# Gaurav14cs17/Bayer_Low_light_Image_Enhancement

Hardware: AMD Instinct MI355X
Metric: megapixels/sec RawFormer-S 512x512 RAW->sRGB (higher is better)
Workload: dtype f32; 1 GPU; RawFormer-S(FLCA) dim=32, batch=8 of packed 4x512x512 synthetic Bayer per GPU; frames_per_gpu=8, variant=flca, weights=synthetic (seeded, random-init scale), parallelism=batch-sharded x1, device=AMD Radeon Graphics

## Files before the change

### bayer_low_light_image_enhancement_amd/_lib.py

```python
from __future__ import annotations

import ctypes as C
import os

_HERE = os.path.dirname(os.path.abspath(__file__))
LIB_PATH = os.environ.get("RF_LIB_PATH") or os.path.join(_HERE, "csrc", "librawformer_hip.so")

RF_VARIANT_FLCA = 0
RF_VARIANT_PLAIN = 1
RF_VARIANT_TRUECOLOR = 2


class RfConfig(C.Structure):
    _fields_ = [("dim", C.c_int32), ("heads", C.c_int32 * 4), ("inp_channels", C.c_int32),
                ("out_channels", C.c_int32), ("ffn_expansion", C.c_int32), ("variant", C.c_int32),
                ("branch_lrelu", C.c_int32), ("clamp_io", C.c_int32), ("flca_levels", C.c_int32)]


_vp, _i, _f, _sz = C.c_void_p, C.c_int, C.c_float, C.c_size_t
ALLREDUCE_FN = C.CFUNCTYPE(None, C.c_void_p, C.c_void_p, C.c_size_t, C.c_int, C.c_void_p)
_psz = C.POINTER(C.c_size_t)
GRAD_READY_FN = C.CFUNCTYPE(None, C.c_void_p, C.c_size_t, C.c_size_t, C.c_void_p)

SIGNATURES = {
    "rf_last_error": (C.c_char_p, []),
    "rf_version": (_i, []),
    "rf_profile_begin": (_i, []),
    "rf_profile_end": (_i, [C.c_char_p, _sz]),
    "rf_create": (_i, [C.POINTER(RfConfig), C.POINTER(_vp)]),
    "rf_destroy": (None, [_vp]),
    "rf_param_count": (_i, [_vp]),
    "rf_param_info": (_i, [_vp, _i, C.POINTER(C.c_char_p), C.POINTER(C.c_int64 * 4), C.POINTER(_i)]),
    "rf_set_param": (_i, [_vp, C.c_char_p, _vp, C.POINTER(C.c_int64), _i]),
    "rf_packed_bytes": (_i, [_vp, _psz]),
    "rf_pack_params": (_i, [_vp, _vp, _sz, _vp]),
    "rf_workspace_bytes": (_i, [_vp, _i, _i, _i, _psz]),
    "rf_forward": (_i, [_vp, _vp, _vp, _vp, _sz, _i, _i, _i, _i, _vp]),
    "rf_forward_stage": (_i, [_vp, _i, _vp, _vp, _vp, _vp, _sz, _i, _i, _i, _vp]),
    "rf_set_shard": (_i, [_vp, _i, _i, _i, ALLREDUCE_FN, _vp]),
    "rf_set_shard_grid": (_i, [_vp, _i, _i, _i, _i, _i, _i, ALLREDUCE_FN, _vp]),
    "rf_flat_param_floats": (_i, [_vp, _psz]),
    "rf_flat_offset": (_i, [_vp, _i, _psz]),
    "rf_train_workspace_bytes": (_i, [_vp, _i, _i, _i, _psz]),
    "rf_set_grad_ready": (_i, [_vp, GRAD_READY_FN, _vp]),
    "rf_set_loss_clamp": (_i, [_vp, _i]),
    "rf_grad_range_count": (_i, [_vp, C.POINTER(_i)]),
    "rf_grad_range": (_i, [_vp, _i, _psz, _psz]),
    "rf_train_step": (_i, [_vp, _vp, _vp, _vp, _vp, _vp, _vp, _sz, _i, _i, _i, _i, _f, _vp]),
    "rf_adam_step": (_i, [_vp, _vp, _vp, _vp, _sz, _f, _f, _f, _f, _f, _i, _i, _f, _vp]),
    "rf_pixel_unshuffle2": (_i, [_vp, _vp, _i, _i, _i, _i, _vp]),
    "rf_pixel_shuffle2": (_i, [_vp, _vp, _i, _i, _i, _i, _vp]),
    "rf_dwt_haar": (_i, [_vp, _vp, _i, _i, _i, _i, _vp]),
    "rf_idwt_haar": (_i, [_vp, _vp, _i, _i, _i, _i, _vp]),
    "rf_dwt_custom": (_i, [_vp, _vp, C.POINTER(C.c_float), _i, _i, _i, _i, _i, _vp]),
    "rf_idwt_custom": (_i, [_vp, _vp, C.POINTER(C.c_float), _i, _i, _i, _i, _i, _vp]),
    "rf_haar_dwt": (_i, [_vp, _vp, _i, _i, _i, _i, _vp]),
    "rf_layernorm2d": (_i, [_vp, _vp, _vp, _vp, _f, _i, _i, _i, _i, _vp]),
    "rf_conv1x1_scratch_bytes": (_i, [_i, _i, _psz]),
    "rf_conv1x1": (_i, [_vp, _vp, _vp, _vp, _vp, _vp, _vp, _vp, _vp, _i, _i, _i, _i, _i, _i, _vp]),
    "rf_dwconv3x3": (_i, [_vp, _vp, _vp, _vp, _i, _i, _i, _i, _i, _vp]),
    "rf_conv3x3_scratch_bytes": (_i, [_i, _i, _psz]),
    "rf_conv3x3": (_i, [_vp, _vp, _vp, _vp, _vp, _i, _i, _i, _i, _i, _i, _i, _vp]),
    "rf_convT2x2_scratch_bytes": (_i, [_i, _i, _psz]),
    "rf_convT2x2": (_i, [_vp, _vp, _vp, _vp, _vp, _i, _i, _i, _i, _i, _vp]),
    "rf_chan_attn_scratch_bytes": (_i, [_i, _i, _i, _i, _i, _psz]),
    "rf_chan_attn": (_i, [_vp] * 10 + [_i] * 5 + [_vp]),
    "rf_transformer_block_scratch_bytes": (_i, [_i, _i, _i, _i, _i, _i, _psz]),
    "rf_transformer_block": (_i, [_vp, _vp, C.POINTER(_vp), _vp, _i, _i, _i, _i, _i, _i, _vp]),
    "rf_flca_scratch_bytes": (_i, [_i, _i, _i, _i, _psz]),
    "rf_flca": (_i, [_vp, _vp, _vp, C.POINTER(_vp), _vp, _i, _i, _i, _i, _vp]),
    "rf_guidance_scratch_bytes": (_i, [_i, _i, _i, _psz]),
    "rf_flca_guidance": (_i, [_vp, _vp, _vp, _i, _i, _i, _i, _i, _vp]),
    "rf_to_uint8_hwc": (_i, [_vp, _vp, _i, _i, _i, _i, _vp]),
    "rf_u8_sse": (_i, [_vp, _vp, _vp, _i, _sz, _vp]),
    "rf_u8_channel_sums": (_i, [_vp, _vp, _i, _i, _sz, _vp]),
    "rf_u8_ssim_scratch_bytes": (_i, [_i, _i, _i, _i, _psz]),
    "rf_u8_ssim": (_i, [_vp, _vp, _vp, _vp, _i, _i, _i, _i, _vp]),
    "rf_sid_pack": (_i, [_vp, _vp, _i, _i, _i, _i, _i, C.c_double, _i, _vp]),
    "rf_sid_check_desc": (_i, [C.POINTER(C.c_int), _i, _i, _i, _i, _i, _i]),
    "rf_sid_sample": (_i, [_vp, _vp, _vp, _vp, _vp, _vp, _i, _i, _i, _i, _i, _i, _i, _i, _vp]),
    "rf_mcr_sample": (_i, [_vp, _vp, _vp, _vp, _vp, _vp, _i, _i, _i, _i, _i, _i, _vp]),
    "rf_token_attn": (_i, [_vp, _vp, _vp, _vp, C.c_longlong, C.c_longlong, _i, _i, _i, _i, _f, _vp]),
    "rf_bayer_luma_scratch_bytes": (_i, [_i, _i, _i, _psz]),
    "rf_bayer_luma": (_i, [_vp, _vp, _vp, _i, _i, _i, _i, _vp]),
    "rf_luma_film_scratch_bytes": (_i, [_i, _i, _i, _psz]),
    "rf_luma_film": (_i, [_vp, _vp, _vp, C.c_longlong, _vp, _vp, _vp, _vp, _i, _i, _i, _i, _vp]),
    "rf_dwgate3x3": (_i, [_vp, _vp, _vp, _vp, _vp, _vp, _i, _i, _i, _i, _vp]),
    "rf_dwconv5x5": (_i, [_vp, _vp, _vp, _vp, _i, _i, _i, _i, _vp]),
    "rf_rfft2_polar_scratch_bytes": (_i, [_i, _i, _i, _psz]),
    "rf_rfft2_polar": (_i, [_vp, _vp, _vp, _vp, _i, _i, _i, _vp]),
    "rf_polar_irfft2": (_i, [_vp, _vp, _vp, _vp, _i, _i, _i, _vp]),
    "rf_feb_scratch_bytes": (_i, [_i, _i, _i, _i, _psz]),
    "rf_feb": (_i, [_vp, _vp, C.POINTER(_vp), _vp, _i, _i, _i, _i, _vp]),
    "rf_ffab_scratch_bytes": (_i, [_i, _i, _i, _i, _psz]),
    "rf_ffab": (_i, [_vp, _vp, C.POINTER(_vp), _vp, _i, _i, _i, _i, _vp]),
    "rf_affine_clamp_add": (_i, [_vp, _vp, _vp, _sz, _f, _f, _f, _f, _vp]),
    "rf_upcat_scratch_bytes": (_i, [_i, _psz]),
    "rf_upcat": (_i, [_vp] * 8 + [_i, _i, _i, _i, _vp]),
}

_lib = None


def load() -> C.CDLL:
    global _lib
    if _lib is None:
        if not os.path.exists(LIB_PATH):
            raise RuntimeError(
                f"{LIB_PATH} not found: build it with `python -m bayer_low_light_image_enhancement_amd.build` "
                "(hipcc, gfx950).  There is no CPU fallback for the RawFormer HIP path.")
        lib = C.CDLL(LIB_PATH)
        for name, (res, args) in SIGNATURES.items():
# ... 12 lines not shown
```

### bayer_low_light_image_enhancement_amd/csrc/rf_api.hip

```cpp
#include <cstdarg>
#include <cstdio>
#include <cstring>
#include <map>
#include <string>
#include <vector>
#include "rf_common.h"

namespace rf {

static thread_local char g_err[512] = "";

void set_error(const char* fmt, ...) {
    va_list ap;
    va_start(ap, fmt);
    vsnprintf(g_err, sizeof(g_err), fmt, ap);
    va_end(ap);
}

int check_hip(hipError_t e, const char* what) {
    if (e == hipSuccess) return RF_OK;
    set_error("%s: %s", what, hipGetErrorString(e));
    return RF_E_DEVICE;
}

// ... 81 lines not shown
    return launch_pixel_unshuffle2(in, out, B, C, h, w, (hipStream_t)stream);
}

int rf_pixel_shuffle2(const float* in, float* out, int B, int C, int h, int w, void* stream) {
    RF_CHECK_ARG(in && out && B > 0 && C > 0 && h > 0 && w > 0, "pixel_shuffle2: bad arguments");
    return launch_pixel_shuffle2(in, out, B, C, h, w, (hipStream_t)stream);
}

int rf_dwt_haar(const float* in, float* out, int B, int C, int h, int w, void* stream) {
    RF_CHECK_ARG(in && out && B > 0 && C > 0 && h > 0 && w > 0, "dwt_haar: bad arguments");
    return launch_dwt2x2(in, out, kHaarInit, 0, 1, B, C, h, w, 2 * h, 2 * w, (hipStream_t)stream);
}

int rf_idwt_haar(const float* in, float* out, int B, int C, int h, int w, void* stream) {
    RF_CHECK_ARG(in && out && B > 0 && C > 0 && h > 0 && w > 0, "idwt_haar: bad arguments");
    return launch_idwt2x2(in, out, kHaarInit, 0, 1, B, C, h, w, (hipStream_t)stream);
}

static void scaled_kernel(const float* k16, int norm, float out[16]) {
    for (int i = 0; i < 16; ++i) out[i] = norm ? k16[i] / 2.0f : k16[i];
}

int rf_dwt_custom(const float* in, float* out, const float* k16, int norm, int B, int C, int h, int w, void* stream) {
    RF_CHECK_ARG(in && out && k16 && B > 0 && C > 0 && h > 0 && w > 0, "dwt_custom: bad arguments");
    float k[16];
    scaled_kernel(k16, norm, k);
    return launch_dwt2x2(in, out, k, 1, 0, B, C, h, w, 2 * h, 2 * w, (hipStream_t)stream);
}

int rf_idwt_custom(const float* in, float* out, const float* k16, int norm, int B, int C, int h, int w, void* stream) {
    RF_CHECK_ARG(in && out && k16 && B > 0 && C > 0 && h > 0 && w > 0, "idwt_custom: bad arguments");
    float k[16];
    scaled_kernel(k16, norm, k);
    return launch_idwt2x2(in, out, k, 1, 0, B, C, h, w, (hipStream_t)stream);
}

int rf_haar_dwt(const float* in, float* out, int B, int C, int hin, int win, void* stream) {
    RF_CHECK_ARG(in && out && B > 0 && C > 0 && hin > 1 && win > 1, "haar_dwt: bad arguments");
    return launch_dwt2x2(in, out, kHaarOrtho, 0, 0, B, C, (hin + 1) / 2, (win + 1) / 2, hin, win, (hipStream_t)stream);
}

int rf_layernorm2d(const float* in, float* out, const float* weight, const float* bias, float eps,
                   int B, int C, int h, int w, void* stream) {
    RF_CHECK_ARG(in && out && weight && B > 0 && C > 0 && h > 0 && w > 0, "layernorm2d: bad arguments");
    return launch_layernorm2d(in, out, weight, bias, eps, B, C, h * w, (hipStream_t)stream);
}

int rf_conv1x1_scratch_bytes(int Cin_total, int Cout, size_t* bytes) {
    RF_CHECK_ARG(bytes && Cin_total > 0 && Cout > 0, "conv1x1_scratch_bytes: bad arguments");
    *bytes = (align_up(packed1x1_floats(Cin_total, Cout), 64) + packed1x1_b3_floats(Cin_total, Cout)) * sizeof(float);
    return RF_OK;
}

int rf_conv1x1(const float* in, const float* in2, float* out, const float* weight, const float* bias,
               const float* ln_w, const float* ln_b, const float* res, void* scratch,
               int B, int C1, int C2, int Cout, int h, int w, void* stream) {
    RF_CHECK_ARG(in && out && weight && scratch && aligned16(scratch), "conv1x1: bad arguments");
    hipStream_t st = (hipStream_t)stream;
    const int K = C1 + C2;
    RF_TRY(pack_1x1(weight, (float*)scratch, Cout, K, K, 1, st));
    float* w3 = (float*)scratch + align_up(packed1x1_floats(K, Cout), 64);
    RF_TRY(pack_1x1_b3(weight, w3, Cout, K, K, 1, st));
    Conv1x1Args a{};
    a.x1 = in; a.C1 = C1; a.x1_bstride = (int64_t)C1 * h * w;
    a.x2 = C2 ? in2 : nullptr; a.C2 = C2; a.x2_bstride = (int64_t)C2 * h * w;
    a.wp = (const float*)scratch; a.wp3 = w3; a.bias = bias; a.ln_w = ln_w; a.ln_b = ln_b; a.ln_eps = 1e-5f;
    a.res = res; a.res_bstride = (int64_t)Cout * h * w;
    a.out = out; a.out_bstride = (int64_t)Cout * h * w; a.Cout = Cout; a.B = B; a.P = h * w; a.w = w;
    return launch_conv1x1(a, st);
}

int rf_dwconv3x3(const float* in, float* out, const float* weight, const float* bias, int gelu,
                 int B, int C, int h, int w, void* stream) {
    RF_CHECK_ARG(in && out && weight && B > 0 && C > 0 && h > 0 && w > 0, "dwconv3x3: bad arguments");
    DwConvArgs a{};
    a.x = in; a.x_bstride = (int64_t)C * h * w; a.out = out; a.out_bstride = (int64_t)C * h * w;
    a.w = weight; a.bias = bias; a.B = B; a.C = C; a.h = h; a.w_ = w; a.gelu = gelu;
    return launch_dwconv3x3(a, (hipStream_t)stream);
}

int rf_conv3x3_scratch_bytes(int Cin, int Cout, size_t* bytes) {
    RF_CHECK_ARG(bytes && Cin > 0 && Cout > 0, "conv3x3_scratch_bytes: bad arguments");
    *bytes = packed3x3_floats(Cin, Cout) * sizeof(float);
    return RF_OK;
}

int rf_conv3x3(const float* in, float* out, const float* weight, const float* bias, void* scratch,
               int act, int store, int B, int Cin, int Cout, int h, int w, void* stream) {
    RF_CHECK_ARG(in && out && weight && scratch && aligned16(scratch), "conv3x3: bad arguments");
    hipStream_t st = (hipStream_t)stream;
    RF_TRY(pack_3x3(weight, (float*)scratch, Cout, Cin, st));
    Conv3x3Args a{};
    a.x = in; a.x_bstride = (int64_t)Cin * h * w; a.wp = (const float*)scratch; a.bias = bias;
    a.out = out; a.out_bstride = (int64_t)Cout * h * w; a.B = B; a.Cin = Cin; a.Cout = Cout; a.h = h; a.w = w;
    a.act = act; a.store = store;
    return launch_conv3x3(a, st);
}

int rf_convT2x2_scratch_bytes(int Cin, int Cout, size_t* bytes) {
    RF_CHECK_ARG(bytes && Cin > 0 && Cout > 0, "convT2x2_scratch_bytes: bad arguments");
    *bytes = packed1x1_floats(Cin, 4 * Cout) * sizeof(float);
    return RF_OK;
}

int rf_convT2x2(const float* in, float* out, const float* weight, const float* bias, void* scratch,
                int B, int Cin, int Cout, int h, int w, void* stream) {
// ... 169 lines not shown
```

### bayer_low_light_image_enhancement_amd/csrc/rf_common.h

```cpp
#pragma once
#include <hip/hip_runtime.h>
#include <stdint.h>
#include <stddef.h>
#include "../../include/rawformer_hip.h"

namespace rf {

typedef float f32x4 __attribute__((ext_vector_type(4)));

void set_error(const char* fmt, ...);
int check_hip(hipError_t e, const char* what);
int check_launch(const char* what);

#define RF_CHECK_ARG(cond, ...)            \
    do {                                   \
        if (!(cond)) {                     \
            rf::set_error(__VA_ARGS__);    \
            return RF_E_INVALID;           \
        }                                  \
    } while (0)

#define RF_TRY(expr)            \
    do {                        \
        const int rc_ = (expr); \
// ... 80 lines not shown
#undef RF_B3
}
#endif

int pack_1x1(const float* w, float* packed, int Cout, int K, int64_t row_stride, int64_t col_stride, hipStream_t st);
int pack_3x3(const float* w, float* packed, int Cout, int Cin, hipStream_t st);
int pack_convT(const float* w, float* packed, int Cin, int Cout, hipStream_t st);

struct PackDesc {
    const float* src; float* dst;
    int kind;
    int rows, cols;
    int64_t rs, cs;
    int flip;
};
constexpr int kPackBatch = 48;
struct PackBatch { PackDesc d[kPackBatch]; };
size_t pack_desc_floats(const PackDesc& d);
int launch_pack_batch(const PackDesc* d, int n, hipStream_t st);

size_t upcat_packed_floats(int C);
int pack_upcat(const float* up_w, const float* up_b, const float* cr_w, const float* cr_b, float* packed, int C, hipStream_t st);
bool upcat_supported(int C, int h, int w, const void* x, const void* skip, const void* out);
int launch_upcat(const float* x, const float* skip, float* out, const float* packed, int B, int C, int h, int w, hipStream_t st);

struct Conv1x1Args {
    const float* x1;
    const float* x2;
    int C1, C2;
    int64_t x1_bstride;
    int64_t x2_bstride;
    const float* x3;
    int C3;
    int64_t x3_bstride;
    const float* wp;
    int64_t wp_bstride;
    const void* wp3;
    int64_t wp3_bstride;
    const float* bias;
    const float* ln_w;
    const float* ln_b;
    float ln_eps;
    const float* res;
    int64_t res_bstride;
    float* out;
    int64_t out_bstride;
    int Cout;
    int B, P;
    int w;
    int mode;
    int act;
};
int launch_conv1x1(const Conv1x1Args& a, hipStream_t st);
bool conv1x1_ln_single_pass(const Conv1x1Args& a);

struct Conv3x3Args {
    const float* x;
    int64_t x_bstride;
    const float* wp;
    const float* bias;
    float* out;
    int64_t out_bstride;
    int B, Cin, Cout, h, w;
    int act;
    int store;
    int unshuffle_in;
    int clamp_in;
    int clamp_out;
    float* ks_scratch = nullptr;
    size_t ks_floats = 0;
};
int launch_conv3x3(const Conv3x3Args& a, hipStream_t st);
size_t conv3x3_ksplit_floats(int B, int Cout, int h, int w);
size_t conv3x3_ksplit_counter_bytes();

template <class T> struct SeGroup { T se1_w, se1_b, se3_w, se3_b; };
template <class T> struct FlcaGroup {
    T alpha, beta, gamma;
    T w_low, w_high, w_chr;
    SeGroup<T> se;
};
typedef SeGroup<const float*> SePrm;
typedef FlcaGroup<const float*> FlcaPrm;
typedef FlcaGroup<float*> FlcaGrad;
static inline int flca_hidden(int C) { return C / 8 > 8 ? C / 8 : 8; }

int launch_layernorm2d(const float* in, float* out, const float* w, const float* b, float eps,
                       int B, int C, int P, hipStream_t st);
struct DwConvArgs {
    const float* x; int64_t x_bstride;
    float* out; int64_t out_bstride;
    const float* w;
    const float* bias;
    int B, C, h, w_;
    int gelu;
    float* out2 = nullptr;
};
int launch_dwconv3x3(const DwConvArgs& a, hipStream_t st);
int launch_pixel_unshuffle2(const float* in, float* out, int B, int C, int h, int w, hipStream_t st);
int launch_pixel_shuffle2(const float* in, float* out, int B, int C, int h, int w, hipStream_t st);
int launch_dwt2x2(const float* in, float* out, const float k[16], int layout, int exact_haar,
                  int B, int C, int h, int w, int hin, int win, hipStream_t st);
int launch_idwt2x2(const float* in, float* out, const float k[16], int layout, int exact_haar,
                   int B, int C, int h, int w, hipStream_t st);

struct GramArgs {
// ... 196 lines not shown
```

### bayer_low_light_image_enhancement_amd/csrc/rf_gemm1x1.hip

```cpp
#include <cstdio>
#include <cstdlib>
#include "rf_common.h"

namespace rf {

__device__ __forceinline__ const float* kset_base(const Conv1x1Args& a, int b, int s) {
    const int k = 4 * s;
    const bool first = k < a.C1;
    const float* src = first ? a.x1 : a.x2;
    const size_t off = (size_t)b * (size_t)(first ? a.x1_bstride : a.x2_bstride) + (size_t)(first ? k : k - a.C1) * (size_t)a.P;
    return src + off;
}

__device__ __forceinline__ float4 ldv(const float* __restrict__ base, unsigned off) {
    return *reinterpret_cast<const float4*>(base + off);
}

template <int NCO, bool RES>
__device__ __forceinline__ void epilogue(const Conv1x1Args& a, f32x4 (&acc)[NCO][4], int tfirst, int ntiles,
                                         const float* __restrict__ bias_l, const float4* res,
                                         int b, int p0, int kq, bool live) {
    const int P = a.P;
    float* outb = a.out + (size_t)b * a.out_bstride;
    if (a.mode == 0) {
// ... 315 lines not shown
    auto chunk = [&](int c, float4 (&xc)[KCH], float4 (&xn)[KCH]) {
        if (c + 1 < nch) {
            load_x_chunk(c + 1, xn);
            load_w_chunk(c + 1);
        }
        const float* wl = &lds_w[c & 1][lane];
#pragma unroll
        for (int i = 0; i < KCH; ++i) {
            float xv[4] = {xc[i].x, xc[i].y, xc[i].z, xc[i].w};
            if constexpr (LN) {
                const int k = 4 * (c * KCH + i) + kq;
                const float gk = gam_l[k], bk = bet_l[k];
#pragma unroll
                for (int g = 0; g < 4; ++g) xv[g] = fmaf(fmaf(xv[g], lnA[g], lnB[g]), gk, bk);
            }
#pragma unroll
            for (int t = 0; t < NCO; ++t) {
                const float av = wl[(i * NCO + t) * 64];
#pragma unroll
                for (int g = 0; g < 4; ++g)
                    acc[t][g] = __builtin_amdgcn_mfma_f32_16x16x4f32(av, xv[g], acc[t][g], 0, 0, 0);
            }
        }
        if (c + 1 < nch) store_w_chunk((c + 1) & 1);
        __syncthreads();
    };

    load_x_chunk(0, xa);
    load_w_chunk(0);
    store_w_chunk(0);
    __syncthreads();
    for (int c = 0; c < nch; c += 2) {
        chunk(c, xa, xb_);
        if (c + 1 < nch) chunk(c + 1, xb_, xa);
    }
    epilogue<NCO, false>(a, acc, t0, tcnt, bias_l, nullptr, b, p0, kq, live);
}


__device__ __forceinline__ void b3_load_x_block(float4 (&xr)[8], const float* xb1, const float* xb2, const float* xb3, int C1, int C2, int C3,
                                                int c, int kq, unsigned P, unsigned pl) {
    const int cb = 32 * c;
    const bool first = cb < C1, third = cb >= C1 + C2;
    const float* src = first ? xb1 : third ? xb3 : xb2;
    const int cloc = first ? cb : third ? cb - C1 - C2 : cb - C1, cmax = (first ? C1 : third ? C3 : C2) - 1;
#pragma unroll
    for (int i = 0; i < 8; ++i) {
        int ch = cloc + 8 * kq + i;
        ch = ch < cmax ? ch : cmax;
        xr[i] = ldv(src, (unsigned)ch * P + pl);
    }
}

template <int NCO, bool LN>
__global__ void __launch_bounds__(256, 2) conv1x1_b3_kernel(Conv1x1Args a, int ngroups) {
    __shared__ __attribute__((aligned(16))) u32x4 lds_w[2][NCO * 3 * 64];
    __shared__ float bias_l[NCO * 16];
    __shared__ float gam_l[LN ? kStreamLnMaxK : 4], bet_l[LN ? kStreamLnMaxK : 4];
    constexpr int WPT = (NCO * 3 * 64 + 255) / 256;
    const int tid = threadIdx.x;
    const int lane = tid & 63, wave = tid >> 6;
    const int j = lane & 15, kq = lane >> 4;
    const int grp = blockIdx.x % ngroups;
    const int tile = blockIdx.x / ngroups;
    const int b = blockIdx.y;
    const int P = a.P;
    const int K = a.C1 + a.C2 + a.C3;
    const int NB = (K + 31) >> 5;
    const int NT = (a.Cout + 15) >> 4;
    const int t0 = grp * NCO;
    const int tcnt = (NT - t0 < NCO) ? NT - t0 : NCO;
    const int p0 = (tile * 4 + wave) * 64 + 4 * j;
    const bool live = p0 < P;
    const unsigned pl = (unsigned)(live ? p0 : 0);
    const u32x4* wp3 = reinterpret_cast<const u32x4*>(reinterpret_cast<const float*>(a.wp3) + (size_t)b * a.wp3_bstride);
    stage_bias(a, bias_l, t0, NCO, tid);
    if constexpr (LN) {
        for (int i = tid; i < 32 * NB; i += 256) {
            gam_l[i] = i < K ? a.ln_w[i] : 0.f;
            bet_l[i] = (a.ln_b && i < K) ? a.ln_b[i] : 0.f;
        }
    }

    f32x4 acc[NCO][4];
#pragma unroll
    for (int t = 0; t < NCO; ++t)
#pragma unroll
        for (int g = 0; g < 4; ++g) acc[t][g] = (f32x4){0.f, 0.f, 0.f, 0.f};
    if (a.res && a.mode == 0) {
        const float* resb = a.res + (size_t)b * a.res_bstride;
#pragma unroll
        for (int t = 0; t < NCO; ++t)
#pragma unroll
            for (int r = 0; r < 4; ++r) {
                const int co = 16 * (t0 + t) + 4 * kq + r;
                const bool ok = live && t < tcnt && co < a.Cout;
                const float4 rv = ldv(resb + (size_t)(ok ? co : 0) * P, pl);
                acc[t][0][r] = ok ? rv.x : 0.f; acc[t][1][r] = ok ? rv.y : 0.f;
                acc[t][2][r] = ok ? rv.z : 0.f; acc[t][3][r] = ok ? rv.w : 0.f;
            }
    }

    float lnA[4] = {1.f, 1.f, 1.f, 1.f}, lnB[4] = {0.f, 0.f, 0.f, 0.f};
    if constexpr (LN) {
        const unsigned voff = (unsigned)kq * (unsigned)P + pl;
        const float4 s4 = ldv(kset_base(a, b, 0), pl);
        const float sh[4] = {s4.x, s4.y, s4.z, s4.w};
        float s1[4] = {0.f, 0.f, 0.f, 0.f}, s2[4] = {0.f, 0.f, 0.f, 0.f};
#pragma unroll 16
        for (int s = 0; s < (K >> 2); ++s) {
            const float4 t = ldv(kset_base(a, b, s), voff);
            const float d[4] = {t.x - sh[0], t.y - sh[1], t.z - sh[2], t.w - sh[3]};
#pragma unroll
            for (int g = 0; g < 4; ++g) { s1[g] += d[g]; s2[g] = fmaf(d[g], d[g], s2[g]); }
        }
        const float invK = 1.0f / (float)K;
#pragma unroll
        for (int g = 0; g < 4; ++g) {
            s1[g] += __shfl_xor(s1[g], 16); s1[g] += __shfl_xor(s1[g], 32);
            s2[g] += __shfl_xor(s2[g], 16); s2[g] += __shfl_xor(s2[g], 32);
            const float md = s1[g] * invK;
            const float var = fmaxf(fmaf(-md, md, s2[g] * invK), 0.f);
            const float rstd = 1.0f / sqrtf(var + a.ln_eps);
            lnA[g] = rstd;
            lnB[g] = a.ln_b ? -(sh[g] + md) * rstd : 0.f;
        }
    }

    float4 xr[8];
    u32x4 wr[WPT];
    const float* const xb1 = a.x1 + (size_t)b * (size_t)a.x1_bstride;
    const float* const xb2 = a.x2 + (size_t)b * (size_t)a.x2_bstride;
    const float* const xb3 = a.x3 + (size_t)b * (size_t)a.x3_bstride;
    auto load_x_block = [&](int c) { b3_load_x_block(xr, xb1, xb2, xb3, a.C1, a.C2, a.C3, c, kq, (unsigned)P, pl); };
    auto load_w_block = [&](int c) {
#pragma unroll
        for (int i = 0; i < WPT; ++i) {
            const int idx = tid + 256 * i;
            const int t = idx / 192, rem = idx - t * 192;
            const bool ok = idx < NCO * 192 && t < tcnt;
            const u32x4 v = wp3[((size_t)c * NT + t0 + (ok ? t : 0)) * 192 + (ok ? rem : 0)];
            wr[i] = ok ? v : (u32x4){0u, 0u, 0u, 0u};
        }
    };
    auto store_w_block = [&](int buf) {
#pragma unroll
        for (int i = 0; i < WPT; ++i)
            if (tid + 256 * i < NCO * 192) lds_w[buf][tid + 256 * i] = wr[i];
    };

    load_x_block(0);
    load_w_block(0);
    store_w_block(0);
    __syncthreads();
    for (int c = 0; c < NB; ++c) {
        u32x4 bp[4][3];
#pragma unroll
        for (int hp = 0; hp < 4; ++hp) {
            float xa[4] = {xr[2 * hp].x, xr[2 * hp].y, xr[2 * hp].z, xr[2 * hp].w};
            float xb[4] = {xr[2 * hp + 1].x, xr[2 * hp + 1].y, xr[2 * hp + 1].z, xr[2 * hp + 1].w};
            if constexpr (LN) {
                const int k = 32 * c + 8 * kq + 2 * hp;
                const float ga = gam_l[k], ba = bet_l[k], gb = gam_l[k + 1], bb = bet_l[k + 1];
#pragma unroll
                for (int g = 0; g < 4; ++g) {
                    xa[g] = fmaf(fmaf(xa[g], lnA[g], lnB[g]), ga, ba);
                    xb[g] = fmaf(fmaf(xb[g], lnA[g], lnB[g]), gb, bb);
                }
            }
#pragma unroll
            for (int g = 0; g < 4; ++g) {
                unsigned a0, a1, a2, b0, b1, b2;
                b3_split(xa[g], a0, a1, a2);
                b3_split(xb[g], b0, b1, b2);
                bp[g][0][hp] = b3_pack(a0, b0);
                bp[g][1][hp] = b3_pack(a1, b1);
                bp[g][2][hp] = b3_pack(a2, b2);
            }
        }
        if (c + 1 < NB) {
            load_x_block(c + 1);
            load_w_block(c + 1);
        }
        const u32x4* wl = &lds_w[c & 1][lane];
#pragma unroll
        for (int t = 0; t < NCO; ++t) {
            const u32x4 ap[3] = {wl[(t * 3 + 0) * 64], wl[(t * 3 + 1) * 64], wl[(t * 3 + 2) * 64]};
            b3_mfma4(ap, bp, acc[t]);
        }
        if (c + 1 < NB) store_w_block((c + 1) & 1);
        __syncthreads();
    }
    epilogue<NCO, false>(a, acc, t0, tcnt, bias_l, nullptr, b, p0, kq, live);
}

template <int KB, int NCO>
__global__ void __launch_bounds__(256, KB <= 4 ? 2 : 1) conv1x1_b3_ln_kernel(Conv1x1Args a, int tpw) {
    __shared__ __attribute__((aligned(16))) u32x4 Bl[KB * 768];
    __shared__ __attribute__((aligned(16))) float red[2 * 4 * 64];
    __shared__ float bias_l[1024];
    constexpr int KPW = KB >= 4 ? KB / 4 : 1;
    constexpr int CPT = KB >= 4 ? 8 : 4;
    constexpr int K = 32 * KB;
    const int tid = threadIdx.x, lane = tid & 63, wave = tid >> 6;
    const int j = lane & 15, kq = lane >> 4;
    const int b = blockIdx.y, P = a.P;
    const int NT = a.Cout >> 4;
    const int ntile = (P + 63) >> 6;
    const float* xb = a.x1 + (size_t)b * a.x1_bstride;
    const u32x4* wp3 = reinterpret_cast<const u32x4*>(reinterpret_cast<const float*>(a.wp3) + (size_t)b * a.wp3_bstride) + lane;
    for (int i = tid; i < a.Cout; i += 256) bias_l[i] = a.bias ? a.bias[i] : 0.f;

    const int kb0 = KB >= 4 ? wave * KPW : wave >> 1;
    const int cbase = KB >= 4 ? 8 * kq : 8 * kq + 4 * (wave & 1);
    float4 xr[KPW][CPT];
    auto load_x = [&](int tile) {
        const int q0 = tile * 64 + 4 * j;
        const unsigned ql = (unsigned)(q0 < P ? q0 : 0);
#pragma unroll
        for (int i = 0; i < KPW; ++i)
#pragma unroll
            for (int c = 0; c < CPT; ++c) xr[i][c] = ldv(xb, (unsigned)(32 * (kb0 + i) + cbase + c) * (unsigned)P + ql);
    };
    constexpr bool PREF = KB != 4;
    if (PREF) load_x(blockIdx.x);
    for (int tile = blockIdx.x; tile < ntile; tile += gridDim.x) {
    if (!PREF) load_x(tile);
    const int p0 = tile * 64 + 4 * j;
    const bool live = p0 < P;
    float mean[4], rstd[4];
    {
        float s[4] = {0.f, 0.f, 0.f, 0.f};
#pragma unroll
        for (int i = 0; i < KPW; ++i)
#pragma unroll
            for (int c = 0; c < CPT; ++c) { s[0] += xr[i][c].x; s[1] += xr[i][c].y; s[2] += xr[i][c].z; s[3] += xr[i][c].w; }
#pragma unroll
        for (int g = 0; g < 4; ++g) { s[g] += __shfl_xor(s[g], 16); s[g] += __shfl_xor(s[g], 32); }
        if (kq == 0) *reinterpret_cast<float4*>(red + wave * 64 + 4 * j) = make_float4(s[0], s[1], s[2], s[3]);
        __syncthreads();
        const float4 r0 = *reinterpret_cast<const float4*>(red + 4 * j), r1 = *reinterpret_cast<const float4*>(red + 64 + 4 * j);
        const float4 r2 = *reinterpret_cast<const float4*>(red + 128 + 4 * j), r3 = *reinterpret_cast<const float4*>(red + 192 + 4 * j);
        mean[0] = (((r0.x + r1.x) + r2.x) + r3.x) * (1.0f / K); mean[1] = (((r0.y + r1.y) + r2.y) + r3.y) * (1.0f / K);
        mean[2] = (((r0.z + r1.z) + r2.z) + r3.z) * (1.0f / K); mean[3] = (((r0.w + r1.w) + r2.w) + r3.w) * (1.0f / K);
        float v[4] = {0.f, 0.f, 0.f, 0.f};
#pragma unroll
// ... 172 lines not shown
    RF_CHECK_ARG(a.C2 == 0 || a.x2 != nullptr, "conv1x1: second source missing");
    RF_CHECK_ARG(a.C3 >= 0 && a.C3 % 4 == 0 && (a.C3 == 0 || (a.x3 != nullptr && a.C2 > 0)), "conv1x1: bad third source (C3 = %d)", a.C3);
    RF_CHECK_ARG(a.mode == 0 || (a.Cout % 4 == 0 && a.w > 0 && a.P % a.w == 0 && !a.res), "conv1x1: bad ConvTranspose geometry");
    RF_CHECK_ARG(a.B <= 65535 && (double)a.P * 4.0 * 16.0 < 4.0e9, "conv1x1: batch %d / plane %d too large", a.B, a.P);
    const int K = a.C1 + a.C2 + a.C3;
    const int NS = K / 4, NT = cdiv(a.Cout, 16);
    bool vec = (a.P % 4 == 0) && aligned16(a.x1) && aligned16(a.out) && (a.x1_bstride % 4 == 0) && (a.out_bstride % 4 == 0);
    if (a.x2) vec = vec && aligned16(a.x2) && (a.x2_bstride % 4 == 0);
    if (a.C3) vec = vec && aligned16(a.x3) && (a.x3_bstride % 4 == 0);
    if (a.res) vec = vec && aligned16(a.res) && (a.res_bstride % 4 == 0);
    if (a.mode == 1) vec = vec && (a.w % 2 == 0);
    const double px = (double)a.B * a.P;
    const double work_flops = 2.0 * K * a.Cout * px, work_bytes = 4.0 * px * (K + a.Cout + (a.res ? a.Cout : 0));
    char key[64];
    bool b3_ok = a.wp3 != nullptr;
#ifdef RF_DIAG
    if (getenv("RF_NO_B3")) b3_ok = false;
#endif
    const bool use_b3 = b3_ok && b3_supported(a);
    RF_CHECK_ARG(a.C3 == 0 || (use_b3 && vec && !a.ln_w && !(a.res && a.Cout % 16 != 0)), "conv1x1: three sources need the bf16x3 kernel (K = %d, P = %d)", K, a.P);
    if (!vec || (a.res && a.Cout % 16 != 0) || (a.ln_w && K > kStreamLnMaxK)) {
        ProfScope prof(st, "conv1x1_scalar_kernel", work_flops, work_bytes);
        int gx = cdiv(a.P, 256);
        if (gx > 4096) gx = 4096;
        conv1x1_scalar_kernel<<<dim3((unsigned)gx, (unsigned)a.B), 256, 0, st>>>(a);
    } else if (int nco_ln = 0; b3_ok && b3_ln_supported(a, &nco_ln)) {
        const int kb = K / 32;
        int tpw = a.Cout / 64;
        const int slots = (kb <= 4 ? 2 : 1) * 256;
        int gx = slots / a.B;
        gx = gx < 1 ? 1 : gx;
        gx = gx < cdiv(a.P, 64) ? gx : cdiv(a.P, 64);
        int zs = 1;
        if ((long)gx * a.B < 128)
            for (int z = tpw / nco_ln; z > 1; --z)
                if ((tpw / nco_ln) % z == 0 && (long)gx * a.B * z <= 512) { zs = z; break; }
        tpw /= zs;
        dim3 grid((unsigned)gx, (unsigned)a.B, (unsigned)zs);
        snprintf(key, sizeof(key), "conv1x1_b3_ln_kernel<%d, %d>", kb, nco_ln);
        ProfScope prof(st, key, work_flops, work_bytes);
        if (kb == 2) {
            if (nco_ln == 3) conv1x1_b3_ln_kernel<2, 3><<<grid, 256, 0, st>>>(a, tpw);
            else conv1x1_b3_ln_kernel<2, 2><<<grid, 256, 0, st>>>(a, tpw);
        } else if (kb == 4) {
            if (nco_ln == 3) conv1x1_b3_ln_kernel<4, 3><<<grid, 256, 0, st>>>(a, tpw);
            else conv1x1_b3_ln_kernel<4, 2><<<grid, 256, 0, st>>>(a, tpw);
        } else {
            if (nco_ln == 4) conv1x1_b3_ln_kernel<8, 4><<<grid, 256, 0, st>>>(a, tpw);
            else if (nco_ln == 3) conv1x1_b3_ln_kernel<8, 3><<<grid, 256, 0, st>>>(a, tpw);
            else conv1x1_b3_ln_kernel<8, 2><<<grid, 256, 0, st>>>(a, tpw);
        }
    } else if (use_b3) {
        int nco = (!a.ln_w && (NT % 6 == 0 || (NT % 4 != 0 && NT > 8))) ? 6 : 4;
        if (!a.ln_w && nco == 4 && NT % 2 == 0 && (long)cdiv(a.P, 256) * cdiv(NT, 4) * a.B < 256) nco = 2;
        const int ngroups = cdiv(NT, nco);
        dim3 grid((unsigned)(cdiv(a.P, 256) * ngroups), (unsigned)a.B, 1);
        snprintf(key, sizeof(key), "conv1x1_b3_kernel<%d, %s>", nco, a.ln_w ? "true" : "false");
        ProfScope prof(st, key, work_flops, work_bytes);
        if (nco == 6) {
            conv1x1_b3_kernel<6, false><<<grid, 256, 0, st>>>(a, ngroups);
        } else if (nco == 2) {
            conv1x1_b3_kernel<2, false><<<grid, 256, 0, st>>>(a, ngroups);
        } else {
            if (a.ln_w) conv1x1_b3_kernel<4, true><<<grid, 256, 0, st>>>(a, ngroups);
            else conv1x1_b3_kernel<4, false><<<grid, 256, 0, st>>>(a, ngroups);
        }
    } else if (NS <= 16 || (NS <= 32 && !a.ln_w && !a.res)) {
        const int ks = NS <= 4 ? 4 : NS <= 8 ? 8 : NS <= 12 ? 12 : NS <= 16 ? 16 : NS <= 24 ? 24 : 32;
        int cap = (240 / ks) & ~1;
        if (a.res && cap > 4) cap = 4;
        if (a.res && (ks <= 8 || a.ln_w) && cap > 2) cap = 2;
        int ntw = NT < cap ? NT : cap;
        const int ngroups = cdiv(NT, ntw);
        const int tpad = cdiv(ntw, 2) * 2;
        const size_t lds = ((size_t)ks * tpad * 64 + tpad * 16 + 8 * ks) * sizeof(float);
        const int slots = 256 * (ks <= 8 ? 3 : 2);
        int wgs = cdiv(slots, a.B * ngroups);
        if (wgs > cdiv(a.P, 256)) wgs = cdiv(a.P, 256);
        dim3 grid((unsigned)(wgs * ngroups), (unsigned)a.B, 1);
        const int rt = ks <= 16 ? (a.res ? (ntw > 2 ? 4 : 2) : 0) : 0;
        const bool dbuf = ks <= 16 && !(ks > 8 && rt == 4);
        snprintf(key, sizeof(key), "conv1x1_res_kernel<%d, %s, %d, %s>", ks, (ks <= 16 && a.ln_w) ? "true" : "false", rt, dbuf ? "true" : "false");
        ProfScope prof(st, key, work_flops, work_bytes);
        switch (ks) {
            case 4: launch_res<4>(a, ntw, ngroups, grid, lds, st); break;
            case 8: launch_res<8>(a, ntw, ngroups, grid, lds, st); break;
            case 12: launch_res<12>(a, ntw, ngroups, grid, lds, st); break;
            case 16: launch_res<16>(a, ntw, ngroups, grid, lds, st); break;
            case 24: launch_res<24>(a, ntw, ngroups, grid, lds, st); break;
            default: launch_res<32>(a, ntw, ngroups, grid, lds, st); break;
        }
    } else {
        int nco = (NT % 8 == 0 || NT > 12) ? 8 : 4;
        if (nco == 8) {
            const long units = (long)cdiv(a.P, 256) * a.B;
            const long cost8 = ((units * cdiv(NT, 8) + 511) / 512) * 8, cost4 = ((units * cdiv(NT, 4) + 511) / 512) * 4;
            if (cost4 < cost8) nco = 4;
        }
        const int ngroups = cdiv(NT, nco);
        dim3 grid((unsigned)(cdiv(a.P, 256) * ngroups), (unsigned)a.B, 1);
        snprintf(key, sizeof(key), "conv1x1_stream_kernel<%d, %d, %s>", nco, nco == 8 ? 4 : 8, a.ln_w ? "true" : "false");
        ProfScope prof(st, key, work_flops, work_bytes);
        if (nco == 8) {
            if (a.ln_w) conv1x1_stream_kernel<8, 4, true><<<grid, 256, 0, st>>>(a, ngroups);
            else conv1x1_stream_kernel<8, 4, false><<<grid, 256, 0, st>>>(a, ngroups);
        } else {
            if (a.ln_w) conv1x1_stream_kernel<4, 8, true><<<grid, 256, 0, st>>>(a, ngroups);
            else conv1x1_stream_kernel<4, 8, false><<<grid, 256, 0, st>>>(a, ngroups);
        }
    }
    return check_launch("conv1x1");
}
// ... 3 lines not shown
```

### include/rawformer_hip.h

```cpp
#ifndef RAWFORMER_HIP_H
#define RAWFORMER_HIP_H

#include <stddef.h>
#include <stdint.h>

#ifdef __cplusplus
extern "C" {
#endif

#define RF_OK 0
#define RF_E_INVALID (-22)
#define RF_E_NOMEM (-12)
#define RF_E_MISSING (-2)
#define RF_E_DEVICE (-5)

#define RF_VARIANT_FLCA 0
#define RF_VARIANT_PLAIN 1
#define RF_VARIANT_TRUECOLOR 2

typedef struct rf_handle rf_handle;

typedef struct rf_config {
    int32_t dim;
    int32_t heads[4];
// ... 7 lines not shown
} rf_config;

const char* rf_last_error(void);
int rf_version(void);

int rf_profile_begin(void);
int rf_profile_end(char* json, size_t len);

int rf_create(const rf_config* cfg, rf_handle** out);
void rf_destroy(rf_handle* h);
int rf_param_count(const rf_handle* h);
int rf_param_info(const rf_handle* h, int index, const char** name, int64_t shape[4], int* ndim);
int rf_set_param(rf_handle* h, const char* name, const float* dev_ptr, const int64_t* shape, int ndim);
int rf_packed_bytes(const rf_handle* h, size_t* bytes);
int rf_pack_params(rf_handle* h, void* packed_dev, size_t bytes, void* stream);
int rf_workspace_bytes(const rf_handle* h, int B, int H, int W, size_t* bytes);
int rf_forward(rf_handle* h, const float* in, float* out, void* workspace, size_t workspace_bytes,
               int B, int H, int W, int packed_input, void* stream);

typedef void (*rf_allreduce_fn)(void* user, float* buf, size_t n, int op, void* stream);
int rf_set_shard(rf_handle* h, int y_lo, int y_hi, int total_rows, rf_allreduce_fn allreduce, void* user);
int rf_set_shard_grid(rf_handle* h, int y_lo, int y_hi, int total_rows, int x_lo, int x_hi, int total_cols,
                      rf_allreduce_fn allreduce, void* user);

int rf_forward_stage(rf_handle* h, int stage, const float* in, const float* packed, float* out, void* workspace,
                     size_t workspace_bytes, int B, int H, int W, void* stream);

int rf_set_loss_clamp(rf_handle* h, int on);
int rf_flat_param_floats(const rf_handle* h, size_t* floats);
int rf_flat_offset(const rf_handle* h, int index, size_t* offset);
int rf_train_workspace_bytes(const rf_handle* h, int B, int H, int W, size_t* bytes);
typedef void (*rf_grad_ready_fn)(void* user, size_t offset, size_t count, void* stream);
int rf_set_grad_ready(rf_handle* h, rf_grad_ready_fn ready, void* user);
int rf_grad_range_count(const rf_handle* h, int* count);
int rf_grad_range(const rf_handle* h, int index, size_t* offset, size_t* count);
int rf_train_step(rf_handle* h, const float* in, const float* gt, float* grads, float* loss_out, float* pred_out, void* workspace,
                  size_t workspace_bytes, int B, int H, int W, int loss_mode, float loss_eps, void* stream);
int rf_adam_step(float* params, const float* grads, float* m, float* v, size_t n, float lr, float beta1, float beta2, float eps,
                 float weight_decay, int decoupled, int step, float grad_scale, void* stream);

int rf_pixel_unshuffle2(const float* in, float* out, int B, int C, int h, int w, void* stream);
int rf_pixel_shuffle2(const float* in, float* out, int B, int C, int h, int w, void* stream);
int rf_dwt_haar(const float* in, float* out, int B, int C, int h, int w, void* stream);
int rf_idwt_haar(const float* in, float* out, int B, int C, int h, int w, void* stream);
int rf_dwt_custom(const float* in, float* out, const float* k16, int norm, int B, int C, int h, int w, void* stream);
int rf_idwt_custom(const float* in, float* out, const float* k16, int norm, int B, int C, int h, int w, void* stream);
int rf_haar_dwt(const float* in, float* out, int B, int C, int hin, int win, void* stream);
int rf_layernorm2d(const float* in, float* out, const float* weight, const float* bias, float eps,
                   int B, int C, int h, int w, void* stream);
int rf_conv1x1_scratch_bytes(int Cin_total, int Cout, size_t* bytes);
int rf_conv1x1(const float* in, const float* in2, float* out, const float* weight, const float* bias,
               const float* ln_w, const float* ln_b, const float* res, void* scratch,
               int B, int C1, int C2, int Cout, int h, int w, void* stream);
int rf_dwconv3x3(const float* in, float* out, const float* weight, const float* bias, int gelu,
                 int B, int C, int h, int w, void* stream);
int rf_conv3x3_scratch_bytes(int Cin, int Cout, size_t* bytes);
int rf_conv3x3(const float* in, float* out, const float* weight, const float* bias, void* scratch,
               int act, int store, int B, int Cin, int Cout, int h, int w, void* stream);
int rf_convT2x2_scratch_bytes(int Cin, int Cout, size_t* bytes);
int rf_convT2x2(const float* in, float* out, const float* weight, const float* bias, void* scratch,
                int B, int Cin, int Cout, int h, int w, void* stream);
int rf_chan_attn_scratch_bytes(int B, int C, int heads, int h, int w, size_t* bytes);
int rf_chan_attn(const float* in, float* out, const float* qkv_w, const float* qkv_b,
                 const float* dw_w, const float* dw_b, const float* temperature,
                 const float* proj_w, const float* proj_b, void* scratch,
                 int B, int C, int heads, int h, int w, void* stream);
int rf_transformer_block_scratch_bytes(int B, int C, int heads, int ffn_expansion, int h, int w, size_t* bytes);
int rf_transformer_block(const float* in, float* out, const float* const* prm, void* scratch,
                         int B, int C, int heads, int ffn_expansion, int h, int w, void* stream);
int rf_flca_scratch_bytes(int B, int C, int h, int w, size_t* bytes);
int rf_flca(const float* feat, const float* guide, float* out, const float* const* prm, void* scratch,
            int B, int C, int h, int w, void* stream);
int rf_guidance_scratch_bytes(int B, int H, int W, size_t* bytes);
int rf_flca_guidance(const float* packed, float* guide, void* scratch, int B, int H, int W, int hf, int wf, void* stream);

int rf_rfft2_polar_scratch_bytes(int planes, int h, int w, size_t* bytes);
int rf_rfft2_polar(const float* in, float* mag, float* pha, void* scratch, int planes, int h, int w, void* stream);
int rf_polar_irfft2(const float* mag, const float* pha, float* out, void* scratch, int planes, int h, int w, void* stream);
int rf_feb_scratch_bytes(int B, int nc, int h, int w, size_t* bytes);
int rf_feb(const float* in, float* out, const float* const* prm, void* scratch, int B, int nc, int h, int w, void* stream);
int rf_ffab_scratch_bytes(int B, int nc, int h, int w, size_t* bytes);
int rf_ffab(const float* in, float* out, const float* const* prm, void* scratch, int B, int nc, int h, int w, void* stream);
int rf_affine_clamp_add(const float* in, const float* add, float* out, size_t n, float scale, float shift, float lo, float hi, void* stream);

int rf_upcat_scratch_bytes(int C, size_t* bytes);
int rf_upcat(const float* x, const float* skip, float* out, const float* up_w, const float* up_b, const float* cr_w, const float* cr_b,
             void* scratch, int B, int C, int h, int w, void* stream);

int rf_to_uint8_hwc(const float* in, unsigned char* out, int B, int C, int h, int w, void* stream);
int rf_u8_sse(const unsigned char* a, const unsigned char* b, unsigned long long* sse, int B, size_t n_per_image, void* stream);
int rf_u8_channel_sums(const unsigned char* a, unsigned long long* sums, int B, int C, size_t hw, void* stream);
int rf_u8_ssim_scratch_bytes(int B, int C, int h, int w, size_t* bytes);
int rf_u8_ssim(const unsigned char* a, const unsigned char* b, double* ssim_sums , void* scratch,
               int B, int C, int h, int w, void* stream);

int rf_sid_pack(const unsigned short* raw, float* out, int B, int h, int w, int black, int white, double ratio, int mode, void* stream);

int rf_sid_check_desc(const int* desc_host, int N, int H, int W, int B, int ph, int pw);
int rf_sid_sample(const unsigned short* raw, const unsigned short* gt, const float* amp, const int* desc, float* x_out, float* gt_out,
                  int N, int H, int W, int B, int ph, int pw, int black, int white, void* stream);

int rf_mcr_sample(const unsigned char* raw, const unsigned char* gt, const double* amp, const int* desc, float* x_out, float* gt_out,
                  int N, int H, int W, int B, int ph, int pw, void* stream);

int rf_token_attn(const float* q, const float* k, const float* v, float* out, long long bstride_qkv, long long bstride_out,
                  int B, int heads, int d, int N, float scale, void* stream);
// ... 15 lines not shown
```

Before: 1021 MP/s.

## Pair two output-channel groups per 512-thread block in conv1x1 b3 kernel

Adds a paired form of the non-LayerNorm conv1x1_b3 kernel. Each 512-thread block runs two output-channel groups over the same pixel tile, and a swizzled block-id map orders tiles in chunks of 8 units across groups to improve cache locality. It is meant to share input-tile loads through L1/L2 and cut block count for large grids. In exchange it doubles the LDS footprint per block, may lower occupancy, and leaves half a block idle when the group count is odd.

```diff
diff --git a/bayer_low_light_image_enhancement_amd/_lib.py b/bayer_low_light_image_enhancement_amd/_lib.py
--- a/bayer_low_light_image_enhancement_amd/_lib.py
+++ b/bayer_low_light_image_enhancement_amd/_lib.py
@@ -58,6 +58,8 @@
     "rf_layernorm2d": (_i, [_vp, _vp, _vp, _vp, _f, _i, _i, _i, _i, _vp]),
     "rf_conv1x1_scratch_bytes": (_i, [_i, _i, _psz]),
     "rf_conv1x1": (_i, [_vp, _vp, _vp, _vp, _vp, _vp, _vp, _vp, _vp, _i, _i, _i, _i, _i, _i, _vp]),
+    "rf_conv1x1_group_grid": (_i, [_i, _i, C.POINTER(_i)]),
+    "rf_conv1x1_group_map": (_i, [_i, _i, _i, C.POINTER(_i), C.POINTER(_i)]),
     "rf_dwconv3x3": (_i, [_vp, _vp, _vp, _vp, _i, _i, _i, _i, _i, _vp]),
     "rf_conv3x3_scratch_bytes": (_i, [_i, _i, _psz]),
     "rf_conv3x3": (_i, [_vp, _vp, _vp, _vp, _vp, _i, _i, _i, _i, _i, _i, _i, _vp]),
diff --git a/bayer_low_light_image_enhancement_amd/csrc/rf_api.hip b/bayer_low_light_image_enhancement_amd/csrc/rf_api.hip
--- a/bayer_low_light_image_enhancement_amd/csrc/rf_api.hip
+++ b/bayer_low_light_image_enhancement_amd/csrc/rf_api.hip
@@ -157,6 +157,22 @@
     return RF_OK;
 }
 
+int rf_conv1x1_group_grid(int units, int ngroups, int* ids) {
+    RF_CHECK_ARG(ids && units > 0 && ngroups > 0 && (long)units * ngroups < (1L << 30), "conv1x1_group_grid: bad arguments");
+    *ids = (int)conv1x1_group_grid((unsigned)units, (unsigned)ngroups);
+    return RF_OK;
+}
+
+int rf_conv1x1_group_map(int units, int ngroups, int id, int* unit, int* group) {
+    RF_CHECK_ARG(unit && group && units > 0 && ngroups > 0 && (long)units * ngroups < (1L << 30) && id >= 0 &&
+                 (unsigned)id < conv1x1_group_grid((unsigned)units, (unsigned)ngroups), "conv1x1_group_map: bad arguments");
+    unsigned u, g;
+    const bool ok = conv1x1_group_map((unsigned)id, (unsigned)units, (unsigned)ngroups, &u, &g);
+    *unit = ok ? (int)u : -1;
+    *group = ok ? (int)g : -1;
+    return RF_OK;
+}
+
 int rf_conv1x1(const float* in, const float* in2, float* out, const float* weight, const float* bias,
                const float* ln_w, const float* ln_b, const float* res, void* scratch,
                int B, int C1, int C2, int Cout, int h, int w, void* stream) {
diff --git a/bayer_low_light_image_enhancement_amd/csrc/rf_common.h b/bayer_low_light_image_enhancement_amd/csrc/rf_common.h
--- a/bayer_low_light_image_enhancement_amd/csrc/rf_common.h
+++ b/bayer_low_light_image_enhancement_amd/csrc/rf_common.h
@@ -156,6 +156,13 @@
     int act;
 };
 int launch_conv1x1(const Conv1x1Args& a, hipStream_t st);
+__host__ __device__ inline bool conv1x1_group_map(unsigned id, unsigned units, unsigned ngroups, unsigned* unit, unsigned* grp) {
+    const unsigned chunk = id / (8u * ngroups), r = id - chunk * 8u * ngroups;
+    *unit = 8u * chunk + (r & 7u);
+    *grp = r >> 3;
+    return *unit < units;
+}
+inline unsigned conv1x1_group_grid(unsigned units, unsigned ngroups) { return (units + 7u) / 8u * 8u * ngroups; }
 bool conv1x1_ln_single_pass(const Conv1x1Args& a);
 
 struct Conv3x3Args {
diff --git a/bayer_low_light_image_enhancement_amd/csrc/rf_gemm1x1.hip b/bayer_low_light_image_enhancement_amd/csrc/rf_gemm1x1.hip
--- a/bayer_low_light_image_enhancement_amd/csrc/rf_gemm1x1.hip
+++ b/bayer_low_light_image_enhancement_amd/csrc/rf_gemm1x1.hip
@@ -391,29 +391,38 @@
     }
 }
 
-template <int NCO, bool LN>
-__global__ void __launch_bounds__(256, 2) conv1x1_b3_kernel(Conv1x1Args a, int ngroups) {
-    __shared__ __attribute__((aligned(16))) u32x4 lds_w[2][NCO * 3 * 64];
-    __shared__ float bias_l[NCO * 16];
+template <int NCO, bool LN, bool PAIR = false>
+__global__ void __launch_bounds__(PAIR ? 512 : 256, 2) conv1x1_b3_kernel(Conv1x1Args a, int ngroups) {
+    static_assert(!(PAIR && LN), "the paired form has no LayerNorm prologue");
+    constexpr int NH = PAIR ? 2 : 1;
+    __shared__ __attribute__((aligned(16))) u32x4 lds_w[NH * 2][NCO * 3 * 64];
+    __shared__ float bias_l[NH * NCO * 16];
     __shared__ float gam_l[LN ? kStreamLnMaxK : 4], bet_l[LN ? kStreamLnMaxK : 4];
     constexpr int WPT = (NCO * 3 * 64 + 255) / 256;
-    const int tid = threadIdx.x;
+    const int tid = PAIR ? threadIdx.x & 255 : threadIdx.x;
+    const int half = PAIR ? threadIdx.x >> 8 : 0;
     const int lane = tid & 63, wave = tid >> 6;
     const int j = lane & 15, kq = lane >> 4;
-    const int grp = blockIdx.x % ngroups;
-    const int tile = blockIdx.x / ngroups;
-    const int b = blockIdx.y;
+    unsigned unit = 0, gp = 0, utiles = 1;
+    if constexpr (PAIR) {
+        utiles = (unsigned)(a.P + 255) >> 8;
+        if (!conv1x1_group_map(blockIdx.x, (unsigned)a.B * utiles, (unsigned)(ngroups + 1) >> 1, &unit, &gp)) return;
+    }
+    const int grp = PAIR ? 2 * (int)gp + half : blockIdx.x % ngroups;
+    const int tile = PAIR ? unit % utiles : blockIdx.x / ngroups;
+    const int b = PAIR ? unit / utiles : blockIdx.y;
     const int P = a.P;
     const int K = a.C1 + a.C2 + a.C3;
     const int NB = (K + 31) >> 5;
     const int NT = (a.Cout + 15) >> 4;
-    const int t0 = grp * NCO;
-    const int tcnt = (NT - t0 < NCO) ? NT - t0 : NCO;
+    const bool idle = PAIR && grp >= ngroups;
+    const int t0 = idle ? 0 : grp * NCO;
+    const int tcnt = idle ? 0 : (NT - t0 < NCO) ? NT - t0 : NCO;
     const int p0 = (tile * 4 + wave) * 64 + 4 * j;
     const bool live = p0 < P;
     const unsigned pl = (unsigned)(live ? p0 : 0);
     const u32x4* wp3 = reinterpret_cast<const u32x4*>(reinterpret_cast<const float*>(a.wp3) + (size_t)b * a.wp3_bstride);
-    stage_bias(a, bias_l, t0, NCO, tid);
+    stage_bias(a, bias_l + half * NCO * 16, t0, NCO, tid);
     if constexpr (LN) {
         for (int i = tid; i < 32 * NB; i += 256) {
             gam_l[i] = i < K ? a.ln_w[i] : 0.f;
@@ -485,7 +494,7 @@
     auto store_w_block = [&](int buf) {
 #pragma unroll
         for (int i = 0; i < WPT; ++i)
-            if (tid + 256 * i < NCO * 192) lds_w[buf][tid + 256 * i] = wr[i];
+            if (tid + 256 * i < NCO * 192) lds_w[2 * half + buf][tid + 256 * i] = wr[i];
     };
 
     load_x_block(0);
@@ -521,7 +530,7 @@
             load_x_block(c + 1);
             load_w_block(c + 1);
         }
-        const u32x4* wl = &lds_w[c & 1][lane];
+        const u32x4* wl = &lds_w[2 * half + (c & 1)][lane];
 #pragma unroll
         for (int t = 0; t < NCO; ++t) {
             const u32x4 ap[3] = {wl[(t * 3 + 0) * 64], wl[(t * 3 + 1) * 64], wl[(t * 3 + 2) * 64]};
@@ -530,7 +539,7 @@
         if (c + 1 < NB) store_w_block((c + 1) & 1);
         __syncthreads();
     }
-    epilogue<NCO, false>(a, acc, t0, tcnt, bias_l, nullptr, b, p0, kq, live);
+    epilogue<NCO, false>(a, acc, t0, tcnt, bias_l + half * NCO * 16, nullptr, b, p0, kq, live);
 }
 
 template <int KB, int NCO>
@@ -809,12 +818,24 @@
         }
     } else if (use_b3) {
         int nco = (!a.ln_w && (NT % 6 == 0 || (NT % 4 != 0 && NT > 8))) ? 6 : 4;
-        if (!a.ln_w && nco == 4 && NT % 2 == 0 && (long)cdiv(a.P, 256) * cdiv(NT, 4) * a.B < 256) nco = 2;
+        const long units = (long)cdiv(a.P, 256) * a.B;
+        bool pair = !a.ln_w && cdiv(NT, nco) > 1 && units * cdiv(cdiv(NT, nco), 2) >= 256;
+#ifdef RF_DIAG
+        if (const char* e = getenv("RF_B3_PAIR")) pair = !a.ln_w && cdiv(NT, nco) > 1 && e[0] != '0';
+#endif
+        if (!pair && !a.ln_w && nco == 4 && NT % 2 == 0 && units * cdiv(NT, 4) < 256) nco = 2;
         const int ngroups = cdiv(NT, nco);
         dim3 grid((unsigned)(cdiv(a.P, 256) * ngroups), (unsigned)a.B, 1);
-        snprintf(key, sizeof(key), "conv1x1_b3_kernel<%d, %s>", nco, a.ln_w ? "true" : "false");
+        const long pair_ids = (units + 7) / 8 * 8 * cdiv(ngroups, 2);
+        RF_CHECK_ARG(!pair || pair_ids < (1L << 31), "conv1x1: %ld pixel tiles x %d output groups is too large a grid", units, ngroups);
+        if (pair) snprintf(key, sizeof(key), "conv1x1_b3_kernel<%d, false, true>", nco);
+        else snprintf(key, sizeof(key), "conv1x1_b3_kernel<%d, %s>", nco, a.ln_w ? "true" : "false");
         ProfScope prof(st, key, work_flops, work_bytes);
-        if (nco == 6) {
+        if (pair) {
+            const unsigned gx = conv1x1_group_grid((unsigned)units, (unsigned)cdiv(ngroups, 2));
+            if (nco == 6) conv1x1_b3_kernel<6, false, true><<<gx, 512, 0, st>>>(a, ngroups);
+            else conv1x1_b3_kernel<4, false, true><<<gx, 512, 0, st>>>(a, ngroups);
+        } else if (nco == 6) {
             conv1x1_b3_kernel<6, false><<<grid, 256, 0, st>>>(a, ngroups);
         } else if (nco == 2) {
             conv1x1_b3_kernel<2, false><<<grid, 256, 0, st>>>(a, ngroups);
diff --git a/include/rawformer_hip.h b/include/rawformer_hip.h
--- a/include/rawformer_hip.h
+++ b/include/rawformer_hip.h
@@ -83,6 +83,8 @@
 int rf_conv1x1(const float* in, const float* in2, float* out, const float* weight, const float* bias,
                const float* ln_w, const float* ln_b, const float* res, void* scratch,
                int B, int C1, int C2, int Cout, int h, int w, void* stream);
+int rf_conv1x1_group_grid(int units, int ngroups, int* ids);
+int rf_conv1x1_group_map(int units, int ngroups, int id, int* unit, int* group);
 int rf_dwconv3x3(const float* in, float* out, const float* weight, const float* bias, int gelu,
                  int B, int C, int h, int w, void* stream);
 int rf_conv3x3_scratch_bytes(int Cin, int Cout, size_t* bytes);
```

New measurement: 1052 MP/s (median of 6 runs). 1.03x the previous value.
